# GATB/bcalm

Measured on AMD Instinct MI355X. Metric: distinct k-mers/s reads->unitigs k=31, higher is better.
Workload: dtype u64; 1 GPU; BASELINE config 3: synthetic 100000000 x 150 bp reads per GPU, k=31, abundance-min 2, 1% substitutions, 30x coverage; multi_gpu=single GPU, minimizer_size=16, log2_partitions=22

## Files before the change

bcalm_amd/csrc/host_glue.h:

```cpp
#pragma once

namespace {

template <int W>
int glue_join_impl(cdbg_ctx* c, bool sharded) {
    if (c->stage < 2) return fail(CDBG_E_STATE, "cdbg_glue before cdbg_compact");
    hipStream_t s = c->stream;
    const uint64_t NP = c->n_pieces;
    if (2 * NP >= 0x7FFFFFF0ULL) return fail(CDBG_E_INTERNAL, "too many pieces for 31-bit end ids (%llu)", (unsigned long long)NP);
    const uint32_t NS = (uint32_t)(2 * NP);
    Timer t; CK(t.start(s));
    CK(c->link.alloc(NS, false));
    HIPCK(hipMemsetAsync(c->link.p, 0xFF, (size_t)std::max<uint32_t>(NS, 1) * sizeof(uint32_t), s));
    HIPCK(hipMemsetAsync(c->dstats.p, 0, 32 * sizeof(uint64_t), s));
    HIPCK(hipMemsetAsync(c->derr.p, 0, 4 * sizeof(uint32_t), s));
    const uint32_t world = sharded ? (uint32_t)c->prm.world_size : 1u;
    const uint64_t n_mine = c->n_glog / world + (world > 1 ? (c->n_glog >> 6) + 1024 : 0);
    bool bucketed = (c->knobs.get("CDBG_GLUE_TABLE") == nullptr || c->direct_join) && c->n_glog > 0;
    if (bucketed && c->direct_join) {
        const uint64_t JB = 1ull << c->join_log_jb;
        JoinBucketParams bp{ c->jfill.p, c->jrecs.p, (uint32_t)JB, c->link.p, c->dstats.p, nullptr, nullptr, 0, nullptr };
        CDBG_LAUNCH((k_join_bucket<W>), std::min<uint64_t>((JB + 3) / 4, 256 * 16), JB_THREADS, s, bp);
    } else if (bucketed) {
        int log_jb = 0; while (((uint64_t)(JB_CAP / 2) << log_jb) < n_mine && log_jb < 26) ++log_jb;
        const uint64_t JB = 1ull << log_jb;
        CK(c->jfill.alloc(JB, false)); CK(c->jrecs.alloc(JB * JB_CAP * (W + 1), false));
        HIPCK(hipMemsetAsync(c->jfill.p, 0, JB * sizeof(uint32_t), s));
        JoinScatterParams sp{ c->glog_keys.p, c->glog_tag.p, c->n_glog, log_jb, c->jfill.p, c->jrecs.p, c->derr.p,
                              world - 1, world > 1 ? (uint32_t)c->prm.rank : 0u };
        CDBG_LAUNCH((k_join_scatter<W>), std::min<uint64_t>((c->n_glog + GLUE_THREADS - 1) / GLUE_THREADS, 1u << 16), GLUE_THREADS, s, sp);
        JoinBucketParams bp{ c->jfill.p, c->jrecs.p, (uint32_t)JB, c->link.p, c->dstats.p, nullptr, nullptr, 0, nullptr };
        CDBG_LAUNCH((k_join_bucket<W>), std::min<uint64_t>((JB + 3) / 4, 256 * 16), JB_THREADS, s, bp);
        HIPCK(hipStreamSynchronize(s));
        uint32_t e = 0; CK(read_u32(c->derr.p, &e));
        if (e == 8) {
            bucketed = false;
            HIPCK(hipMemsetAsync(c->link.p, 0xFF, (size_t)std::max<uint32_t>(NS, 1) * sizeof(uint32_t), s));
            HIPCK(hipMemsetAsync(c->dstats.p, 0, 32 * sizeof(uint64_t), s));
            HIPCK(hipMemsetAsync(c->derr.p, 0, 4 * sizeof(uint32_t), s));
        }
    }
    if (!bucketed && c->n_glog) {
        CK(glue_table_slots(n_mine + n_mine / 4 + 1024, &c->glue_cap));
        CK(c->glue_keys.alloc((uint64_t)c->glue_cap * W, false));
        CK(c->glue_a.alloc(c->glue_cap, false)); CK(c->glue_b.alloc(c->glue_cap, false)); CK(c->glue_conf.alloc(c->glue_cap, false));
        HIPCK(hipMemsetAsync(c->glue_keys.p, 0xFF, (uint64_t)c->glue_cap * W * sizeof(uint64_t), s));
        HIPCK(hipMemsetAsync(c->glue_a.p, 0, (uint64_t)c->glue_cap * sizeof(uint32_t), s));
        HIPCK(hipMemsetAsync(c->glue_b.p, 0, (uint64_t)c->glue_cap * sizeof(uint32_t), s));
        HIPCK(hipMemsetAsync(c->glue_conf.p, 0, (uint64_t)c->glue_cap * sizeof(uint32_t), s));
        GlueBuildParams bp{ c->glog_keys.p, c->glog_tag.p, c->n_glog, c->glue_keys.p, c->glue_a.p, c->glue_b.p, c->glue_conf.p, c->glue_cap - 1,
                            world - 1, world > 1 ? (uint32_t)c->prm.rank : 0u };
        CDBG_LAUNCH((k_glue_build<W>), std::min<uint64_t>((c->n_glog + GLUE_THREADS - 1) / GLUE_THREADS, MAX_GRID), GLUE_THREADS, s, bp);
        GlueResolveParams gp{};
        gp.keys = c->glue_keys.p; gp.a = c->glue_a.p; gp.b = c->glue_b.p; gp.conf = c->glue_conf.p;
        gp.cap = c->glue_cap; gp.W = W; gp.link = c->link.p; gp.stats = c->dstats.p;
        CDBG_LAUNCH(k_glue_resolve, std::min<uint64_t>((c->glue_cap + GLUE_THREADS - 1) / GLUE_THREADS, GLUE_RESOLVE_GRID), GLUE_THREADS, s, gp);
    }
    float ms = 0; CK(t.stop(&ms));
    CK(check_device_error(c, "glue join"));
    uint64_t gs = 0; CK(read_u64(c->dstats.p, &gs));
    c->n_join_local = gs; c->st.ms_glue = ms; c->joined = true;
    return CDBG_OK;
}


int glue_walk(cdbg_ctx* c, bool* done) {
    hipStream_t s = c->stream;
    const uint64_t NP = c->n_pieces, NS = 2 * NP;
    *done = false;
    if (!NP) return CDBG_OK;
    const uint64_t ucap = std::max<uint64_t>(NP, 1);
    const uint64_t ocap = std::max<uint64_t>(c->n_piece_bases, 1);
    CK(c->unitig_off.alloc(ucap, false)); CK(c->unitig_len.alloc(ucap, false)); CK(c->unitig_kc.alloc(ucap, false));
    CK(c->unitig_bases.alloc(ocap + 64, false));
    if (c->prm.all_abundance_counts) CK(c->unitig_ab.alloc(ocap, false));
    CK(c->rank_flag.alloc(4, true));
    CK(c->walk_rec.alloc(NS, false)); CK(c->walk_heads.alloc(NS, false)); CK(c->walk_hlen.alloc(NS, false)); CK(c->walk_hoff.alloc(NS, false));
    HIPCK(hipMemsetAsync(c->cursors.p + 2, 0, 2 * sizeof(uint64_t), s));
    HIPCK(hipMemsetAsync(c->dstats.p, 0, 32 * sizeof(uint64_t), s));
    HIPCK(hipMemsetAsync(c->derr.p, 0, 4 * sizeof(uint32_t), s));
    HIPCK(hipMemsetAsync(c->rank_flag.p, 0, sizeof(uint32_t), s));
    uint32_t max_steps = 4096;
    if (const char* e = c->knobs.get("CDBG_WALK_MAX")) max_steps = (uint32_t)strtoul(e, nullptr, 10);
    uint64_t* const n_heads = c->dstats.p + 6;
    WalkInitParams ip{ (uint32_t)NP, c->piece_n.p, c->piece_kc.p, c->piece_boff.p, c->link.p, c->walk_rec.p, c->walk_heads.p, n_heads, c->dstats.p + 4 };
    CDBG_LAUNCH(k_walk_init, (NP + WALK_PIECES - 1) / WALK_PIECES, WALK_THREADS, s, ip);
    const uint64_t spans = (NS + WALK_SPAN - 1) / WALK_SPAN, wave_grid = (spans + WALK_THREADS / 64 - 1) / (WALK_THREADS / 64);
    WalkMeasureParams mp{ c->walk_rec.p, c->walk_heads.p, n_heads, c->walk_hlen.p, max_steps, c->rank_flag.p };
    CDBG_LAUNCH(k_walk_measure, wave_grid, WALK_THREADS, s, mp);
    WalkPlaceParams pp{ n_heads, c->walk_hlen.p, c->walk_hoff.p, c->k, c->cursors.p + 2, c->cursors.p + 3, ucap, ocap, c->derr.p,
                        c->unitig_off.p, c->unitig_len.p };
    CDBG_LAUNCH(k_walk_place, spans, WALK_THREADS, s, pp);
    WalkCopyParams wp{};
    wp.k = c->k; wp.rec = c->walk_rec.p; wp.piece_bases = c->piece_bases.p;
    wp.heads = c->walk_heads.p; wp.n_heads = n_heads; wp.hlen = c->walk_hlen.p; wp.hoff = c->walk_hoff.p;
    wp.unitig_len = c->unitig_len.p; wp.unitig_kc = c->unitig_kc.p; wp.out = c->unitig_bases.p; wp.visited = c->dstats.p + 5;
    wp.piece_ab = c->prm.all_abundance_counts ? c->piece_ab.p : nullptr; wp.unitig_ab = c->unitig_ab.p; wp.error = c->derr.p;
    if (c->k >= 9) CDBG_LAUNCH(k_walk_copy<true>, wave_grid, WALK_THREADS, s, wp);
    else CDBG_LAUNCH(k_walk_copy<false>, wave_grid, WALK_THREADS, s, wp);
    HIPCK(hipStreamSynchronize(s));
    uint64_t d[2]; CK(read_u64(c->dstats.p + 4, d, 2));
    uint32_t gave_up = 0; CK(read_u32(c->rank_flag.p, &gave_up));
    if (gave_up || d[1] != d[0]) { c->walk_off = true; return CDBG_OK; }
    *done = true;
    return CDBG_OK;
}

template <int W>
int glue_impl(cdbg_ctx* c) {
    if (c->stage < 2) return fail(CDBG_E_STATE, "cdbg_glue before cdbg_compact");
    if ((c->prm.world_size > 1 || c->force_multi) && c->have_tr && !c->xchg_done && !c->joined) {
        if (!c->prm.emit_replicated && c->knobs.get("CDBG_GLUE_REPLICATED") == nullptr) {
            const int rc = glue_sharded<W>(c);
            if (rc != DG_FALLBACK) return rc;
        }
        CK(glue_exchange(c));
    }
    if (!c->joined) CK(glue_join_impl<W>(c, false));
    hipStream_t s = c->stream;
    const uint64_t NP = c->n_pieces;
    const uint32_t NS = (uint32_t)(2 * NP);
    const float ms_join = c->st.ms_glue;
    HostMarks hm;
    Timer t; CK(t.start(s));
    bool walked = false;
    if (c->prm.world_size <= 1 && !c->force_multi && !c->xchg_done && !c->walk_off && c->knobs.get("CDBG_GLUE_RANK") == nullptr) CK(glue_walk(c, &walked));
    if (walked) {
        { uint64_t cur[2]; CK(read_u64(c->cursors.p + 2, cur, 2)); c->n_unitigs = cur[0]; c->unitig_total = cur[1]; }
        CK(pack_unitigs(c));
        float ms_fin = 0; CK(t.stop(&ms_fin));
        hm.mark("glue: walk + copy");
        c->st.ms_glue = ms_join + ms_fin;
        CK(check_device_error(c, "glue"));
        c->joined = false;
        c->st.n_glue_joined = c->n_join_local; c->st.n_unitigs = c->n_unitigs; c->st.unitig_bases = c->unitig_total; c->st.n_walked_unitigs = c->n_unitigs;
        c->st.ms_total += c->st.ms_glue;
        c->stage = 3;
        return CDBG_OK;
    }
    DBuf<uint32_t>& flag = c->rank_flag; DBuf<uint4>& st_a = c->rank_a; DBuf<uint4>& st_b = c->rank_b;
    CK(st_a.alloc(NS, false)); CK(st_b.alloc(NS, false));
    CK(flag.alloc(4, true));
    HIPCK(hipMemsetAsync(c->dstats.p, 0, 32 * sizeof(uint64_t), s));
    HIPCK(hipMemsetAsync(c->derr.p, 0, 4 * sizeof(uint32_t), s));
    uint32_t* const link_p = c->link.p;

    uint64_t n_cycles_cut = 0;
    const uint32_t gridS = (NS + GLUE_THREADS - 1) / GLUE_THREADS;
    RankParams rp{};
    uint4* fa_st = nullptr;
    const uint2* st8 = nullptr; uint4* hinfo = nullptr;
    bool ranked = false;
    if (NS) {
        int max_rounds8 = 2; while ((1ull << (max_rounds8 - 1)) < NS) ++max_rounds8;
        Rank8Params r8{ NS, link_p, c->piece_n.p, reinterpret_cast<uint2*>(st_b.p), flag.p };
        CDBG_LAUNCH(k_rank8_init, gridS, GLUE_THREADS, s, r8);
        for (int r = 0; r < max_rounds8 && !ranked; ++r) {
            HIPCK(hipMemsetAsync(flag.p, 0, sizeof(uint32_t), s));
            CDBG_LAUNCH(k_rank8_jump, gridS, GLUE_THREADS, s, r8);
            HIPCK(hipStreamSynchronize(s));
            uint32_t ch = 0; CK(read_u32(flag.p, &ch));
            if (!ch) ranked = true;
        }
        if (ranked) { st8 = r8.a; hinfo = st_a.p; }
    }
    if (NS && !ranked) {
        int max_rounds = 2; while ((1ull << (max_rounds - 1)) < NS) ++max_rounds;
        for (int pass = 0; pass < 2; ++pass) {
            rp.n_states = NS; rp.link = link_p; rp.piece_n = c->piece_n.p;
            rp.st_a = st_a.p; rp.st_b = st_b.p; rp.changed = flag.p;
            CDBG_LAUNCH(k_rank_init, gridS, GLUE_THREADS, s, rp);
            bool converged = false;
            for (int r = 0; r < max_rounds; ++r) {
                HIPCK(hipMemsetAsync(flag.p, 0, sizeof(uint32_t), s));
                CDBG_LAUNCH(k_rank_jump, gridS, GLUE_THREADS, s, rp);
                std::swap(rp.st_a, rp.st_b);
                HIPCK(hipStreamSynchronize(s));
                uint32_t ch = 0; CK(read_u32(flag.p, &ch));
                if (!ch) { converged = true; break; }
            }
            fa_st = rp.st_a;
            if (converged) break;
            if (pass == 1) return fail(CDBG_E_INTERNAL, "list ranking did not converge after cutting cycles");
            HIPCK(hipMemsetAsync(flag.p, 0, sizeof(uint32_t), s));
            CutParams cu{ NS, rp.st_a, link_p, flag.p };
            CDBG_LAUNCH(k_cut_cycles, gridS, GLUE_THREADS, s, cu);
            HIPCK(hipStreamSynchronize(s));
            uint32_t nc = 0; CK(read_u32(flag.p, &nc)); n_cycles_cut += nc;
        }
    }
    if (NS && !st8) {
        uint4* const other = (fa_st == st_a.p) ? st_b.p : st_a.p;
        RankNarrowParams np{ NS, fa_st, reinterpret_cast<uint2*>(other) };
        CDBG_LAUNCH(k_rank_narrow, gridS, GLUE_THREADS, s, np);
        st8 = reinterpret_cast<const uint2*>(other); hinfo = fa_st;
    }
    const uint64_t ucap = std::max<uint64_t>(NP, 1);
    const uint64_t ocap = std::max<uint64_t>(c->n_piece_bases, 1);
    CK(c->unitig_off.alloc(ucap, false)); CK(c->unitig_len.alloc(ucap, false)); CK(c->unitig_kc.alloc(ucap, false));
    CK(c->unitig_bases.alloc(ocap + 64, false));
    if (c->prm.all_abundance_counts) CK(c->unitig_ab.alloc(ocap, false));
    HIPCK(hipMemsetAsync(c->cursors.p + 2, 0, 2 * sizeof(uint64_t), s));
    if (NS) {
        HeadParams hp{};
        hp.n_states = NS; hp.k = c->k; hp.link = link_p; hp.st = st8; hp.hinfo = hinfo;
        hp.unitig_off = c->unitig_off.p; hp.unitig_len = c->unitig_len.p; hp.unitig_kc = c->unitig_kc.p;
        hp.unitig_cap = ucap; hp.out_cap = ocap; hp.n_unitigs = c->cursors.p + 2; hp.out_cursor = c->cursors.p + 3; hp.error = c->derr.p;
        hp.own_lo = 0; hp.own_hi = NS;
        if (c->prm.world_size > 1 && !c->prm.emit_replicated && c->xchg_done) { hp.own_lo = (uint32_t)(2 * c->piece_lo); hp.own_hi = (uint32_t)(2 * c->piece_hi); }
        CDBG_LAUNCH(k_unitig_heads, (NS + HEADS_PER_WG - 1) / HEADS_PER_WG, GLUE_THREADS, s, hp);
        EmitParams ep{};
        ep.n_pieces = (uint32_t)NP; ep.k = c->k; ep.st = st8; ep.hinfo = hp.hinfo;
        ep.piece_n = c->piece_n.p; ep.piece_kc = c->piece_kc.p; ep.piece_boff = c->piece_boff.p; ep.piece_bases = c->piece_bases.p;
        ep.unitig_kc = c->unitig_kc.p; ep.out = c->unitig_bases.p;
        ep.piece_ab = c->prm.all_abundance_counts ? c->piece_ab.p : nullptr; ep.unitig_ab = c->unitig_ab.p;
        CDBG_LAUNCH(k_emit, (uint32_t)((NP + GLUE_THREADS - 1) / GLUE_THREADS), GLUE_THREADS, s, ep);
    }
    { uint64_t cur[2]; CK(read_u64(c->cursors.p + 2, cur, 2)); c->n_unitigs = cur[0]; c->unitig_total = cur[1]; }
    CK(pack_unitigs(c));
    float ms_fin = 0; CK(t.stop(&ms_fin));
    hm.mark("glue: rank + heads + emit");
    c->st.ms_glue = ms_join + ms_fin;
    CK(check_device_error(c, "glue"));
    c->joined = false;
    c->st.n_glue_joined = c->n_join_local; c->st.n_unitigs = c->n_unitigs; c->st.unitig_bases = c->unitig_total; c->st.n_cycles += n_cycles_cut;
    c->st.ms_total += c->st.ms_glue;
    c->stage = 3;
    return CDBG_OK;
}

struct UnitigView { uint64_t U; const uint64_t* off; const uint32_t* len; const uint8_t* bases; uint64_t total_bases; };

template <int W>
int links_build(cdbg_ctx* c, const UnitigView& v, DBuf<uint64_t>& link_off, DBuf<uint32_t>& link_to, uint64_t& n_links) {
    hipStream_t s = c->stream;
    const uint64_t U = v.U, NE = 2 * U;
    if (pow2_at_least(4 * U + 64) > (1ull << 30)) return fail(CDBG_E_INTERNAL, "too many unitigs (%llu) for the 30-bit slots of the link table", (unsigned long long)U);
    const uint32_t cap = (uint32_t)pow2_at_least(4 * U + 64);
    DBuf<uint64_t> lk_keys; DBuf<uint32_t> lk_cnt, lk_ends, end_slot, deg;
    CK(lk_keys.alloc((uint64_t)cap * W, false)); CK(lk_cnt.alloc((uint64_t)cap * 2, true));
    CK(lk_ends.alloc((uint64_t)cap * 2 * LINK_PER_FLAG, false)); CK(end_slot.alloc(NE, false)); CK(deg.alloc(NE, false));
    HIPCK(hipMemsetAsync(lk_keys.p, 0xFF, (uint64_t)cap * W * sizeof(uint64_t), s));
    CK(link_off.alloc(NE + 1, true));
    LinkParams lp{};
    lp.n_unitigs = U; lp.k = c->k; lp.unitig_off = v.off; lp.unitig_len = v.len; lp.bases = v.bases;
    lp.lk_keys = lk_keys.p; lp.lk_cnt = lk_cnt.p; lp.lk_ends = lk_ends.p; lp.lk_mask = cap - 1;
    lp.end_slot = end_slot.p; lp.deg = deg.p;
    n_links = 0;
    if (NE) {
        const uint64_t grid = (NE + LINK_THREADS - 1) / LINK_THREADS;
        CDBG_LAUNCH((k_link_insert<W>), grid, LINK_THREADS, s, lp);
        CDBG_LAUNCH(k_link_count, grid, LINK_THREADS, s, lp);
        const uint64_t nb = (NE + EXSCAN_BLOCK - 1) / EXSCAN_BLOCK;
        CK(c->exscan_tmp.alloc(nb + 1, false));
        const uint32_t* degp = deg.p;
        uint64_t* const loff = link_off.p;
        CDBG_LAUNCH(k_exscan_sums, nb, EXSCAN_THREADS, s, degp, c->exscan_tmp.p, NE);
        CDBG_LAUNCH(k_exscan_top, 1, EXSCAN_THREADS, s, c->exscan_tmp.p, nb, loff + NE);
        CDBG_LAUNCH(k_exscan_apply, nb, EXSCAN_THREADS, s, degp, (const uint64_t*)c->exscan_tmp.p, loff, NE);
        CK(read_u64(loff + NE, &n_links));
        CK(link_to.alloc(n_links, false));
        lp.link_off = link_off.p; lp.link_to = link_to.p;
        CDBG_LAUNCH(k_link_fill, grid, LINK_THREADS, s, lp);
        HIPCK(hipStreamSynchronize(s));
    }
    return CDBG_OK;
}
UnitigView resident_unitigs(cdbg_ctx* c) { return UnitigView{ c->n_unitigs, c->unitig_off.p, c->unitig_len.p, c->unitig_bases.p, c->unitig_total }; }
inline bool holds_a_share(const cdbg_ctx* c) { return (c->prm.world_size > 1 || c->force_multi) && !c->prm.emit_replicated; }

template <int W>
int links_build_sharded(cdbg_ctx* c) {
    hipStream_t s = c->stream;
    const int world = c->prm.world_size, me = c->prm.rank;
    if (!c->have_tr) return fail(CDBG_E_STATE, "cdbg_link on a sharded unitig set needs the transport");
    const uint64_t U = c->n_unitigs, NE = 2 * U;
    std::vector<uint64_t> all(world); const uint64_t mine = U;
    if (c->tr.all_gather_u64(c->tr.user, &mine, all.data(), 1) != 0) return fail(CDBG_E_INTERNAL, "transport all_gather_u64 failed");
    uint64_t tot = 0, base = 0; for (int r = 0; r < world; ++r) { if (r == me) base = tot; tot += all[r]; }
    c->unitig_id_base = base; c->unitig_id_total = tot;
    const uint64_t NA = 2 * tot;
    int rc = CDBG_OK;
    DBuf<uint64_t> lk_keys, end_keys, all_keys; DBuf<uint32_t> lk_cnt, lk_ends, end_slot, deg, end_meta, all_meta;
    uint32_t cap = 0;
    auto local = [&]() -> int {
        if (NA >= (1ull << 31) || pow2_at_least(2 * NA + 64) > (1ull << 30)) return fail(CDBG_E_INTERNAL, "too many unitigs (%llu) for the 30-bit slots of the link table", (unsigned long long)tot);
        cap = (uint32_t)pow2_at_least(2 * NA + 64);
        CK(end_keys.alloc(NE * W + 1, false)); CK(end_meta.alloc(NE + 1, false)); CK(all_keys.alloc(NA * W + 1, false)); CK(all_meta.alloc(NA + 1, false));
        CK(lk_keys.alloc((uint64_t)cap * W, false)); CK(lk_cnt.alloc((uint64_t)cap * 2, true));
        CK(lk_ends.alloc((uint64_t)cap * 2 * LINK_PER_FLAG, false)); CK(end_slot.alloc(NA + 1, false)); CK(deg.alloc(NE + 1, false));
        HIPCK(hipMemsetAsync(lk_keys.p, 0xFF, (uint64_t)cap * W * sizeof(uint64_t), s));
        CK(c->link_off.alloc(NE + 1, true));
        return CDBG_OK;
    };
    rc = local();
    CK(agree(c, rc, "links: buffers"));
    LinkParams lp{};
    lp.n_unitigs = U; lp.k = c->k; lp.unitig_off = c->unitig_off.p; lp.unitig_len = c->unitig_len.p; lp.bases = c->unitig_bases.p;
    lp.lk_keys = lk_keys.p; lp.lk_cnt = lk_cnt.p; lp.lk_ends = lk_ends.p; lp.lk_mask = cap - 1;
    lp.end_slot = end_slot.p; lp.deg = deg.p; lp.end_keys = end_keys.p; lp.end_meta = end_meta.p;
    lp.all_keys = all_keys.p; lp.all_meta = all_meta.p; lp.n_all_ends = NA; lp.e0 = 2 * base;
    const uint64_t grid = (NE + LINK_THREADS - 1) / LINK_THREADS;
    if (NE) CDBG_LAUNCH((k_link_describe<W>), grid, LINK_THREADS, s, lp);
    std::vector<uint64_t> roff(world), rcnt(world);
    { uint64_t o = 0; for (int r = 0; r < world; ++r) { roff[r] = o * 2 * W * 8; rcnt[r] = all[r] * 2 * W * 8; o += all[r]; } }
    if (!c->tr_ordered) HIPCK(hipStreamSynchronize(s));
    if (c->tr.all_gather_v(c->tr.user, end_keys.p, NE * W * 8, all_keys.p, roff.data(), rcnt.data()) != 0) return fail(CDBG_E_INTERNAL, "transport all_gather_v failed");
    { uint64_t o = 0; for (int r = 0; r < world; ++r) { roff[r] = o * 2 * 4; rcnt[r] = all[r] * 2 * 4; o += all[r]; if (r != me) c->comm_bytes += (NE + 2 * all[r]) * (uint64_t)(W * 8 + 4); } }
    if (c->tr.all_gather_v(c->tr.user, end_meta.p, NE * 4, all_meta.p, roff.data(), rcnt.data()) != 0) return fail(CDBG_E_INTERNAL, "transport all_gather_v failed");
    c->n_links = 0;
    auto join = [&]() -> int {
        if (NA) CDBG_LAUNCH((k_link_insert_described<W>), (NA + LINK_THREADS - 1) / LINK_THREADS, LINK_THREADS, s, lp);
        if (NE) {
            CDBG_LAUNCH(k_link_count, grid, LINK_THREADS, s, lp);
            const uint64_t nb = (NE + EXSCAN_BLOCK - 1) / EXSCAN_BLOCK;
            CK(c->exscan_tmp.alloc(nb + 1, false));
            const uint32_t* degp = deg.p; uint64_t* const loff = c->link_off.p;
            CDBG_LAUNCH(k_exscan_sums, nb, EXSCAN_THREADS, s, degp, c->exscan_tmp.p, NE);
            CDBG_LAUNCH(k_exscan_top, 1, EXSCAN_THREADS, s, c->exscan_tmp.p, nb, loff + NE);
            CDBG_LAUNCH(k_exscan_apply, nb, EXSCAN_THREADS, s, degp, (const uint64_t*)c->exscan_tmp.p, loff, NE);
            CK(read_u64(loff + NE, &c->n_links));
            CK(c->link_to.alloc(c->n_links, false));
            lp.link_off = c->link_off.p; lp.link_to = c->link_to.p;
            CDBG_LAUNCH(k_link_fill, grid, LINK_THREADS, s, lp);
        }
        HIPCK(hipStreamSynchronize(s));
        return CDBG_OK;
    };
    rc = join();
    CK(agree(c, rc, "links: join"));
    return CDBG_OK;
}

template <int W>
int link_impl(cdbg_ctx* c) {
    if (c->stage < 3) return fail(CDBG_E_STATE, "cdbg_link before cdbg_glue");
    if (holds_a_share(c)) CK(links_build_sharded<W>(c));
    else { CK(links_build<W>(c, resident_unitigs(c), c->link_off, c->link_to, c->n_links)); c->unitig_id_base = 0; c->unitig_id_total = c->n_unitigs; }
    c->linked = true;
    return CDBG_OK;
}

template <int W>
int verify_view(cdbg_ctx* c, const UnitigView& v, const uint64_t* link_off, const uint32_t* link_to, bool with_links, uint64_t* out) {
    hipStream_t s = c->stream;
    DBuf<uint64_t> d; CK(d.alloc(8, true));
    VerifyParams vp{ v.U, c->k, v.off, v.len, v.bases,
                     c->seg_off.p, c->seg_n.p, c->solid_keys.p, c->solid_cnt.p, c->n_local_parts, link_off, link_to, d.p };
    if (v.U) CDBG_LAUNCH((k_verify_unitig_kmers<W>), std::min<uint64_t>((v.U + 255) / 256, 1u << 16), 256, s, vp);
    CDBG_LAUNCH((k_verify_solid<W>), std::min<uint64_t>((c->n_local_parts + 255) / 256, 1u << 16), 256, s, vp);
    if (with_links && v.U) CDBG_LAUNCH(k_verify_maximal, (2 * v.U + 255) / 256, 256, s, vp);
    HIPCK(hipStreamSynchronize(s));
    CK(read_u64(d.p, out, 8));
    if (!with_links) out[6] = out[7] = ~0ull;
    return CDBG_OK;
}
template <int W>
int verify_edges_view(cdbg_ctx* c, const UnitigView& v, uint64_t n_links, uint64_t* out) {
    hipStream_t s = c->stream;
    const uint64_t n_home = c->st.n_solid;
    const uint64_t cap = pow2_at_least(3 * n_home + 1024);
    if (cap > (1ull << 32)) return fail(CDBG_E_NOMEM, "too many solid k-mers (%llu) for the 32-bit slots of the junction table", (unsigned long long)n_home);
    DBuf<uint64_t> jt_keys, d; DBuf<uint32_t> jt_cnt;
    CK(jt_keys.alloc(cap * W, false)); CK(jt_cnt.alloc(cap, false)); CK(d.alloc(4, true));
    HIPCK(hipMemsetAsync(jt_keys.p, 0xFF, cap * W * sizeof(uint64_t), s));
    HIPCK(hipMemsetAsync(jt_cnt.p, 0, cap * sizeof(uint32_t), s));
    VerifyEdgeParams ep{ c->k, c->seg_off.p, c->seg_n.p, c->solid_keys.p, c->solid_cnt.p, c->n_local_parts, jt_keys.p, jt_cnt.p, (uint32_t)(cap - 1), d.p };
    CDBG_LAUNCH((k_verify_edge_insert<W>), std::min<uint64_t>((c->n_local_parts + 255) / 256, 1u << 16), 256, s, ep);
    CDBG_LAUNCH(k_verify_edge_sum, std::min<uint64_t>((cap + 255) / 256, 1u << 16), 256, s, ep);
    HIPCK(hipStreamSynchronize(s));
    uint64_t r[4]; CK(read_u64(d.p, r, 4));
    if (r[2]) return fail(CDBG_E_INTERNAL, "junction table overflow in cdbg_verify_edges (%llu ends lost)", (unsigned long long)r[2]);
    out[0] = r[0]; out[1] = n_links; out[2] = 2 * (v.total_bases - v.U * (uint64_t)c->k); out[3] = r[1];
    return CDBG_OK;
}

template <int W>
int verify_impl(cdbg_ctx* c, uint64_t* out) {
    if (c->stage < 3) return fail(CDBG_E_STATE, "cdbg_verify before cdbg_glue");
    const bool sharded_set = holds_a_share(c);
    if (!sharded_set && !c->linked) CK(link_impl<W>(c));
    return verify_view<W>(c, resident_unitigs(c), c->link_off.p, c->link_to.p, !sharded_set, out);
}
template <int W>
int verify_edges_impl(cdbg_ctx* c, uint64_t* out) {
    if (c->stage < 3) return fail(CDBG_E_STATE, "cdbg_verify_edges before cdbg_glue");
    if (c->prm.world_size > 1 || c->force_multi) { out[0] = out[1] = out[2] = out[3] = ~0ull; return CDBG_OK; }
    if (!c->linked) CK(link_impl<W>(c));
    return verify_edges_view<W>(c, resident_unitigs(c), c->n_links, out);
}
template <int W>
int verify_unitigs_impl(cdbg_ctx* c, const char* bases, const uint64_t* off, uint64_t n, uint64_t* out) {
    if (c->stage < 1) return fail(CDBG_E_STATE, "cdbg_verify_unitigs before cdbg_count");
    if (c->prm.world_size > 1 || c->force_multi) return fail(CDBG_E_STATE, "cdbg_verify_unitigs needs the whole solid set on this rank");
    const uint64_t total = n ? off[n] : 0;
    std::vector<uint32_t> len(std::max<uint64_t>(n, 1));
    for (uint64_t i = 0; i < n; ++i) {
        if (off[i + 1] < off[i] || off[i + 1] - off[i] < (uint64_t)c->k || off[i + 1] - off[i] > 0xFFFFFFFFull) return fail(CDBG_E_PARAM, "unitig %llu: bad length", (unsigned long long)i);
        len[i] = (uint32_t)(off[i + 1] - off[i]);
    }
    for (uint64_t i = 0; i < total; ++i) if (!base_valid((uint8_t)bases[i])) return fail(CDBG_E_PARAM, "unitig base %llu is not one of ACGT", (unsigned long long)i);
    DBuf<uint64_t> d_off, l_off; DBuf<uint32_t> d_len, l_to; DBuf<uint8_t> d_bases;
    CK(d_off.alloc(n + 1, false)); CK(d_len.alloc(n, false)); CK(d_bases.alloc(total + 64, false));
    HIPCK(hipMemcpy(d_off.p, off, (n + 1) * sizeof(uint64_t), hipMemcpyHostToDevice));
    HIPCK(hipMemcpy(d_len.p, len.data(), std::max<uint64_t>(n, 1) * sizeof(uint32_t), hipMemcpyHostToDevice));
    if (total) HIPCK(hipMemcpy(d_bases.p, bases, total, hipMemcpyHostToDevice));
    const UnitigView v{ n, d_off.p, d_len.p, d_bases.p, total };
    uint64_t nl = 0;
    CK(links_build<W>(c, v, l_off, l_to, nl));
    CK(verify_view<W>(c, v, l_off.p, l_to.p, true, out));
    return verify_edges_view<W>(c, v, nl, out + 8);
}

}
```

bcalm_amd/csrc/k_walk.h:

```cpp
#pragma once
#include "k_glue.h"

namespace cdbg {

constexpr int WALK_THREADS = 256;
constexpr int WALK_PPT = 8;
constexpr int WALK_PIECES = WALK_THREADS * WALK_PPT;
constexpr int WALK_SPAN = 1024;
constexpr int WALK_SPT = WALK_SPAN / WALK_THREADS;

struct WalkInitParams { uint32_t n_pieces; const uint32_t* piece_n; const uint64_t* piece_kc; const uint64_t* piece_boff; const uint32_t* link;
                        uint4* rec; uint32_t* heads; uint64_t* n_heads; uint64_t* n_live; };
__global__ void __launch_bounds__(WALK_THREADS) k_walk_init(WalkInitParams P) {
    CDBG_SHARED uint32_t s_wn[WALK_THREADS / 64], s_wl[WALK_THREADS / 64]; CDBG_SHARED uint64_t s_base;
    const int tid = threadIdx.x, lane = tid & 63, wave = tid >> 6;
    const uint32_t p0 = blockIdx.x * (uint32_t)WALK_PIECES + (uint32_t)wave * (64u * WALK_PPT) + (uint32_t)lane;
    uint32_t hs[2 * WALK_PPT], at[WALK_PPT]; uint32_t run = 0, live = 0;
#pragma unroll
    for (int i = 0; i < WALK_PPT; ++i) {
        const uint32_t p = p0 + 64u * (uint32_t)i;
        hs[2 * i] = NONE32; hs[2 * i + 1] = NONE32;
        uint32_t cnt = 0;
        if (p < P.n_pieces) {
            const uint32_t n = P.piece_n[p];
            uint4 a, b; a.x = NONE32; a.y = NONE32; a.z = n; a.w = 0; b.x = 0; b.y = 0; b.z = 0; b.w = 0;
            if (n) {
                const uint64_t kc = P.piece_kc[p], bo = P.piece_boff[p];
                const uint2 l = reinterpret_cast<const uint2*>(P.link)[p];
                a.x = l.y; a.y = l.x;
                a.w = (uint32_t)kc; b.x = (uint32_t)(kc >> 32); b.y = (uint32_t)bo; b.z = (uint32_t)(bo >> 32);
                ++live;
                if (l.x == NONE32) { hs[2 * i] = 2 * p; ++cnt; }
                if (l.y == NONE32) { hs[2 * i + 1] = 2 * p + 1; ++cnt; }
            }
            P.rec[2 * (uint64_t)p] = a; P.rec[2 * (uint64_t)p + 1] = b;
        }
        const uint32_t incl = wave_incl_sum_u32(cnt);
        at[i] = run + incl - cnt;
        run += wave_readlane_u32(incl, 63);
    }
    const uint32_t lsum = wave_readlane_u32(wave_incl_sum_u32(live), 63);
    if (lane == 0) { s_wn[wave] = run; s_wl[wave] = lsum; }
    __syncthreads();
    uint32_t wbase = 0, tot = 0, ltot = 0;
    for (int w = 0; w < WALK_THREADS / 64; ++w) { if (w < wave) wbase += s_wn[w]; tot += s_wn[w]; ltot += s_wl[w]; }
    if (tid == 0) {
        s_base = tot ? atomic_add_u64(P.n_heads, (uint64_t)tot) : 0ull;
        if (ltot) atomic_add_u64(P.n_live, (uint64_t)ltot);
    }
    __syncthreads();
    uint32_t* const out = P.heads + s_base + wbase;
#pragma unroll
    for (int i = 0; i < WALK_PPT; ++i) {
        uint32_t j = at[i];
        if (hs[2 * i] != NONE32) out[j++] = hs[2 * i];
        if (hs[2 * i + 1] != NONE32) out[j] = hs[2 * i + 1];
    }
}

CDBG_DEV void walk_copy(const uint8_t* src, uint8_t* dst, uint32_t nb, uint32_t skip, bool fwd) {
    uint32_t i = skip;
    if (nb - skip >= 8u) {
        for (;;) {
            if (i + 8u > nb) { if (i == nb) break; i = nb - 8u; }
            const uint64_t w = fwd ? ld_unaligned_u64(src + i) : comp_ascii8_rev(ld_unaligned_u64(src + (nb - 8u - i)));
            st_unaligned_u64(dst + i, w);
            i += 8u;
        }
    } else {
        uint64_t w = 0; const uint32_t r = nb - skip;
        for (uint32_t j = 0; j < r; ++j) w |= (uint64_t)(fwd ? src[skip + j] : comp_ascii(src[nb - 1 - skip - j])) << (8 * j);
        if (r & 4u) { st_unaligned_u32(dst + i, (uint32_t)w); w >>= 32; i += 4u; }
        if (r & 2u) { st_unaligned_u16(dst + i, (uint16_t)w); w >>= 16; i += 2u; }
        if (r & 1u) dst[i] = (uint8_t)w;
    }
}

CDBG_DEV uint32_t walk_lane_rank(uint64_t mask, int lane) { return (uint32_t)__popcll(mask & ((1ULL << lane) - 1ULL)); }

struct WalkMeasureParams { const uint4* rec; const uint32_t* heads; const uint64_t* n_heads; uint32_t* hlen; uint32_t max_steps; uint32_t* giveup; };
__global__ void __launch_bounds__(WALK_THREADS) k_walk_measure(WalkMeasureParams P) {
    const int lane = threadIdx.x & 63;
    const uint64_t n_heads = *P.n_heads;
    const uint64_t wv = ((uint64_t)blockIdx.x * WALK_THREADS + threadIdx.x) >> 6;
    uint64_t next = wv * WALK_SPAN; const uint64_t end = next + WALK_SPAN < n_heads ? next + WALK_SPAN : n_heads;
    bool active = false; uint32_t e = 0, h = 0, len = 0, steps = 0; uint64_t idx = 0;
    for (;;) {
        const uint64_t need = __ballot(!active);
        if (next < end) {
            const uint64_t my = next + walk_lane_rank(need, lane);
            if (!active && my < end) { idx = my; h = P.heads[my]; e = h; len = 0; steps = 0; active = true; }
            next += (uint64_t)__popcll(need);
        }
        if (!__any(active)) break;
        if (active) {
            const uint4 a = P.rec[2 * (uint64_t)(e >> 1)];
            len += a.z;
            const uint32_t nx = (e & 1u) ? a.y : a.x;
            if (nx == NONE32) { P.hlen[idx] = e > (h ^ 1u) ? len : 0u; active = false; }
            else if (++steps > P.max_steps) { *P.giveup = 1u; P.hlen[idx] = 0u; active = false; }
            else e = nx;
        }
    }
}

struct WalkPlaceParams { const uint64_t* n_heads; uint32_t* hlen; uint64_t* hoff; int k; uint64_t* n_unitigs; uint64_t* out_cursor; uint64_t unitig_cap, out_cap; uint32_t* error;
                         uint64_t* unitig_off; uint32_t* unitig_len; };
__global__ void __launch_bounds__(WALK_THREADS) k_walk_place(WalkPlaceParams P) {
    CDBG_SHARED uint32_t s_wn[WALK_THREADS / 64]; CDBG_SHARED uint64_t s_wl[WALK_THREADS / 64];
    CDBG_SHARED uint64_t s_ubase, s_obase;
    const int tid = threadIdx.x, lane = tid & 63, wave = tid >> 6;
    const uint64_t n_heads = *P.n_heads;
    if ((uint64_t)blockIdx.x * WALK_SPAN >= n_heads) return;
    const uint64_t i0 = (uint64_t)blockIdx.x * WALK_SPAN + (uint64_t)tid * WALK_SPT;
    uint32_t kl[WALK_SPT]; uint32_t kn = 0; uint64_t ksum = 0;
#pragma unroll
    for (int i = 0; i < WALK_SPT; ++i) {
        kl[i] = i0 + i < n_heads ? P.hlen[i0 + i] : 0u;
        if (kl[i]) { ++kn; ksum += (uint64_t)kl[i] + (uint64_t)P.k - 1u; }
    }
    uint32_t icnt = kn; uint64_t isum = ksum;
#pragma unroll
    for (int d = 1; d < 64; d <<= 1) {
        const uint32_t c = __shfl_up(icnt, (unsigned)d); const uint64_t l = __shfl_up(isum, (unsigned)d);
        if (lane >= d) { icnt += c; isum += l; }
    }
    if (lane == 63) { s_wn[wave] = icnt; s_wl[wave] = isum; }
    __syncthreads();
    uint32_t my_i = icnt - kn, tot_n = 0; uint64_t my_o = isum - ksum, tot_l = 0;
    for (int w = 0; w < WALK_THREADS / 64; ++w) {
        if (w < wave) { my_i += s_wn[w]; my_o += s_wl[w]; }
        tot_n += s_wn[w]; tot_l += s_wl[w];
    }
    if (tid == 0 && tot_n) {
        s_ubase = atomic_add_u64(P.n_unitigs, (uint64_t)tot_n);
        s_obase = atomic_add_u64(P.out_cursor, tot_l);
        if (s_ubase + tot_n > P.unitig_cap || s_obase + tot_l > P.out_cap) *P.error = 4;
    }
    __syncthreads();
    if (!tot_n) return;
    const bool fits = s_ubase + tot_n <= P.unitig_cap && s_obase + tot_l <= P.out_cap;
    uint64_t uid = s_ubase + my_i, off = s_obase + my_o;
#pragma unroll
    for (int i = 0; i < WALK_SPT; ++i) {
        if (!kl[i]) continue;
        const uint32_t len = kl[i] + (uint32_t)P.k - 1u;
        P.hlen[i0 + i] = fits ? (uint32_t)uid + 1u : 0u; P.hoff[i0 + i] = off;
        if (fits) { P.unitig_off[uid] = off; P.unitig_len[uid] = len; }
        ++uid; off += (uint64_t)len;
    }
}

struct WalkCopyParams {
    int k; const uint4* rec; const uint8_t* piece_bases;
    const uint32_t* heads; const uint64_t* n_heads; const uint32_t* hlen; const uint64_t* hoff;
    const uint32_t* unitig_len; uint64_t* unitig_kc; uint8_t* out; uint64_t* visited;
    const uint32_t* piece_ab; uint32_t* unitig_ab;
    uint32_t* error;
};

struct WalkWin { uint64_t lo, hi, prev; uint32_t st; };
struct WalkDst { uint8_t* out; uint64_t u0; uint32_t ulen; uint32_t* error; uint32_t flushes; };

CDBG_DEV void wc_guard(WalkDst& D, uint64_t at, uint32_t bytes) {
#ifdef CDBG_HOSTSIM
    if (at < D.u0 || at + bytes > D.u0 + D.ulen) *D.error = 10;
#endif
}
CDBG_DEV void wc_st16(WalkDst& D, uint64_t at, uint64_t lo, uint64_t hi) {
    wc_guard(D, at, 16);
#ifdef CDBG_HOSTSIM
    if (at & 15u) *D.error = 10;
    __builtin_memcpy(D.out + at, &lo, 8); __builtin_memcpy(D.out + at + 8, &hi, 8);
#else
    uint4 v; v.x = (uint32_t)lo; v.y = (uint32_t)(lo >> 32); v.z = (uint32_t)hi; v.w = (uint32_t)(hi >> 32);
    *reinterpret_cast<uint4*>(D.out + at) = v;
#endif
}
CDBG_DEV void wc_st8(WalkDst& D, uint64_t at, uint64_t w) { wc_guard(D, at, 8); st_unaligned_u64(D.out + at, w); }
CDBG_DEV uint64_t wc_bytes8(uint64_t a, uint64_t b, uint32_t r) { return r == 0u ? a : r == 8u ? b : (a >> (8u * r)) | (b << (64u - 8u * r)); }
CDBG_DEV void wc_store_small(WalkDst& D, uint64_t at, uint64_t w0, uint64_t w1, uint64_t w2, uint32_t n) {
    wc_st8(D, at, w0);
    if (n >= 16u) { wc_st8(D, at + 8u, w1); if (n > 16u) wc_st8(D, at + n - 8u, wc_bytes8(w1, w2, n - 16u)); }
    else wc_st8(D, at + n - 8u, wc_bytes8(w0, w1, n - 8u));
}
CDBG_DEV void wc_flush(WalkWin& B, WalkDst& D, uint64_t cb) {
    ++D.flushes;
    if (cb >= D.u0) {
        wc_st16(D, cb, B.lo, B.hi);
        if (B.st == 1u) { const uint32_t h = 16u - ((uint32_t)D.u0 & 15u); wc_st8(D, D.u0, B.prev | (B.lo << (8u * h))); }
        B.prev = B.hi; B.st = 2u;
    } else {
        const uint32_t a = (uint32_t)(D.u0 - cb);
        if (a <= 8u) { wc_st8(D, D.u0, wc_bytes8(B.lo, B.hi, a)); if (a < 8u) wc_st8(D, cb + 8u, B.hi); B.prev = B.hi; B.st = 2u; }
        else { B.prev = B.hi >> (8u * (a - 8u)); B.st = 1u; }
    }
}
CDBG_DEV void wc_append(WalkWin& B, WalkDst& D, uint64_t pos, uint64_t w, uint32_t c) {
    const uint32_t s = (uint32_t)pos & 15u;
    if (s < 8u) { B.lo |= w << (8u * s); if (s) B.hi |= w >> (64u - 8u * s); }
    else {
        const uint32_t s8 = s - 8u;
        B.hi |= w << (8u * s8);
        if (s + c >= 16u) { wc_flush(B, D, pos - s); B.lo = s8 ? w >> (64u - 8u * s8) : 0ull; B.hi = 0; }
    }
}
CDBG_DEV void wc_finish(WalkWin& B, WalkDst& D, uint64_t end) {
    const uint32_t t = (uint32_t)end & 15u;
    if (B.st == 2u) {
        if (t >= 8u) { wc_st8(D, end - t, B.lo); if (t > 8u) wc_st8(D, end - 8u, wc_bytes8(B.lo, B.hi, t - 8u)); }
        else if (t) wc_st8(D, end - 8u, wc_bytes8(B.prev, B.lo, t));
    } else if (B.st == 1u) {
        const uint32_t h = 16u - ((uint32_t)D.u0 & 15u);
        wc_store_small(D, D.u0, B.prev | (B.lo << (8u * h)), (B.lo >> (64u - 8u * h)) | (B.hi << (8u * h)), B.hi >> (64u - 8u * h), h + t);
    } else {
        const uint32_t a = (uint32_t)D.u0 & 15u;
        wc_store_small(D, D.u0, wc_bytes8(B.lo, B.hi, a), B.hi >> (8u * a), 0, (uint32_t)(end - D.u0));
    }
}

template <bool CHUNKED>
__global__ void __launch_bounds__(WALK_THREADS) k_walk_copy(WalkCopyParams P) {
    const int lane = threadIdx.x & 63;
    const uint64_t n_heads = *P.n_heads;
    const uint64_t wv = ((uint64_t)blockIdx.x * WALK_THREADS + threadIdx.x) >> 6;
    uint64_t next = wv * WALK_SPAN; const uint64_t end = next + WALK_SPAN < n_heads ? next + WALK_SPAN : n_heads;
    bool active = false; uint32_t e = 0, koff = 0, uid = 0, seen = 0; uint64_t kc = 0, uoff = 0;
    WalkWin B{ 0, 0, 0, 0 }; WalkDst D{ P.out, 0, 0, P.error, 0 };
    for (;;) {
        const uint64_t need = __ballot(!active);
        if (next < end) {
            const uint64_t my = next + walk_lane_rank(need, lane);
            if (!active && my < end) {
                const uint32_t u1 = P.hlen[my];
                if (u1) {
                    uid = u1 - 1u; uoff = P.hoff[my]; e = P.heads[my]; koff = 0; kc = 0; active = true;
                    B.lo = 0; B.hi = 0; B.st = 0; D.u0 = uoff;
#ifdef CDBG_HOSTSIM
                    D.ulen = P.unitig_len[uid];
#endif
                }
            }
            next += (uint64_t)__popcll(need);
        }
        if (!__any(active)) { if (next < end) continue; break; }
        if (active) {
            const uint32_t p = e >> 1;
            const uint4 a = P.rec[2 * (uint64_t)p], b = P.rec[2 * (uint64_t)p + 1];
            const uint32_t n = a.z, nb = n + (uint32_t)P.k - 1u;
            const uint64_t boff = (uint64_t)b.y | ((uint64_t)b.z << 32);
            kc += (uint64_t)a.w | ((uint64_t)b.x << 32);
            const bool fwd = (e & 1u) == END_LEFT;
            const uint32_t skip = koff ? (uint32_t)P.k - 1u : 0u;
            if constexpr (CHUNKED) {
                const uint8_t* const src = P.piece_bases + boff;
                uint64_t pos = uoff + koff + skip;
                D.flushes = 0;
                for (uint32_t i = skip; i < nb;) {
                    const uint32_t c = nb - i < 8u ? nb - i : 8u, j = i + c - 8u;
                    const uint64_t w = fwd ? ld_unaligned_u64(src + j) : comp_ascii8_rev(ld_unaligned_u64(src + (nb - 8u - j)));
                    wc_append(B, D, pos, w >> (8u * (8u - c)), c);
                    pos += c; i += c;
                }
#ifdef CDBG_HOSTSIM
                if (const char* tf = getenv("CDBG_SIM_WALK_TRACE")) if (FILE* fp = fopen(tf, "a")) {
                    fprintf(fp, "%u %llu %u %u %d %u %d\n", uid, (unsigned long long)uoff, koff + skip, nb - skip, fwd ? 1 : 0, D.flushes,
                            ((e & 1u) ? a.y : a.x) == NONE32 ? 1 : 0);
                    fclose(fp);
                }
#endif
            } else {
#ifdef CDBG_HOSTSIM
                wc_guard(D, uoff + koff + skip, nb - skip);
#endif
                walk_copy(P.piece_bases + boff, P.out + uoff + koff, nb, skip, fwd);
            }
            if (P.piece_ab) {
                const uint32_t* sa = P.piece_ab + boff + (P.k - 1);
                uint32_t* da = P.unitig_ab + uoff + koff + (P.k - 1);
                if (fwd) { for (uint32_t t = 0; t < n; ++t) da[t] = sa[t]; }
                else { for (uint32_t t = 0; t < n; ++t) da[t] = sa[n - 1 - t]; }
            }
            koff += n; ++seen;
            const uint32_t nx = (e & 1u) ? a.y : a.x;
            if (nx == NONE32) {
                if constexpr (CHUNKED) wc_finish(B, D, uoff + koff + (uint32_t)P.k - 1u);
                P.unitig_kc[uid] = kc; active = false;
            }
            else e = nx;
        }
    }
    const uint64_t s64 = wave_sum_u64((uint64_t)seen);
    if (lane == 0 && s64) atomic_add_u64(P.visited, s64);
}

}
```

Baseline: 25.27 billion kmers/s.

## Inline short piece bases as 2-bit packed data in walk records

During walk init, pieces of up to 60 bases (k>=9, no abundance output) are packed into 2-bit form and stored in the 16-byte walk record, with a flag bit and 7 high k-count bits. The copy kernel then expands these inline bases, reverse-complementing in the 2-bit domain when needed, instead of doing scattered unaligned loads from piece_bases. The aim is to cut random global memory reads in the pointer-chasing walk, at the cost of extra bit-manipulation ALU work and more work in the init kernel.

New measurement: 25.46 billion kmers/s (median of 3 runs). About the same (+0.8%).

```diff
diff --git a/bcalm_amd/csrc/host_glue.h b/bcalm_amd/csrc/host_glue.h
--- a/bcalm_amd/csrc/host_glue.h
+++ b/bcalm_amd/csrc/host_glue.h
@@ -83,7 +83,9 @@
     uint32_t max_steps = 4096;
     if (const char* e = c->knobs.get("CDBG_WALK_MAX")) max_steps = (uint32_t)strtoul(e, nullptr, 10);
     uint64_t* const n_heads = c->dstats.p + 6;
-    WalkInitParams ip{ (uint32_t)NP, c->piece_n.p, c->piece_kc.p, c->piece_boff.p, c->link.p, c->walk_rec.p, c->walk_heads.p, n_heads, c->dstats.p + 4 };
+    const uint32_t inline_ok = c->k >= 9 && !c->prm.all_abundance_counts;
+    WalkInitParams ip{ (uint32_t)NP, c->piece_n.p, c->piece_kc.p, c->piece_boff.p, c->link.p, c->walk_rec.p, c->walk_heads.p, n_heads, c->dstats.p + 4,
+                       c->k, c->piece_bases.p, inline_ok };
     CDBG_LAUNCH(k_walk_init, (NP + WALK_PIECES - 1) / WALK_PIECES, WALK_THREADS, s, ip);
     const uint64_t spans = (NS + WALK_SPAN - 1) / WALK_SPAN, wave_grid = (spans + WALK_THREADS / 64 - 1) / (WALK_THREADS / 64);
     WalkMeasureParams mp{ c->walk_rec.p, c->walk_heads.p, n_heads, c->walk_hlen.p, max_steps, c->rank_flag.p };
diff --git a/bcalm_amd/csrc/k_walk.h b/bcalm_amd/csrc/k_walk.h
--- a/bcalm_amd/csrc/k_walk.h
+++ b/bcalm_amd/csrc/k_walk.h
@@ -9,8 +9,36 @@
 constexpr int WALK_SPAN = 1024;
 constexpr int WALK_SPT = WALK_SPAN / WALK_THREADS;
 
+constexpr uint32_t WALK_INLINE = 0x80000000u;
+constexpr uint32_t WALK_INLINE_NB = 60;
+constexpr int WALK_INLINE_KC_BITS = 39;
+CDBG_DEV uint64_t walk_pack8(uint64_t w) {
+    uint64_t x = (w >> 1) & 0x0303030303030303ull;
+    x = (x | (x >> 6)) & 0x000F000F000F000Full;
+    x = (x | (x >> 12)) & 0x000000FF000000FFull;
+    return (x | (x >> 24)) & 0xFFFFull;
+}
+CDBG_DEV uint64_t walk_expand8(uint32_t v) {
+    uint64_t x = v;
+    x = (x | (x << 24)) & 0x000000FF000000FFull;
+    x = (x | (x << 12)) & 0x000F000F000F000Full;
+    x = (x | (x << 6)) & 0x0303030303030303ull;
+    const uint64_t b0 = x & 0x0101010101010101ull, b1 = (x >> 1) & 0x0101010101010101ull, t = b1 & ~b0;
+    return 0x4040404040404040ull | (b0 << 1) | (b1 << 2) | (t << 4) | (t ^ 0x0101010101010101ull);
+}
+CDBG_DEV uint64_t walk_rev2(uint64_t x) {
+    x = ((x >> 2) & 0x3333333333333333ull) | ((x & 0x3333333333333333ull) << 2);
+    x = ((x >> 4) & 0x0F0F0F0F0F0F0F0Full) | ((x & 0x0F0F0F0F0F0F0F0Full) << 4);
+    return __builtin_bswap64(x);
+}
+CDBG_DEV void walk_shr128(uint64_t& lo, uint64_t& hi, uint32_t s) {
+    if (s >= 64u) { lo = hi >> (s - 64u); hi = 0; }
+    else if (s) { lo = (lo >> s) | (hi << (64u - s)); hi >>= s; }
+}
+
 struct WalkInitParams { uint32_t n_pieces; const uint32_t* piece_n; const uint64_t* piece_kc; const uint64_t* piece_boff; const uint32_t* link;
-                        uint4* rec; uint32_t* heads; uint64_t* n_heads; uint64_t* n_live; };
+                        uint4* rec; uint32_t* heads; uint64_t* n_heads; uint64_t* n_live;
+                        int k; const uint8_t* piece_bases; uint32_t inline_ok; };
 __global__ void __launch_bounds__(WALK_THREADS) k_walk_init(WalkInitParams P) {
     CDBG_SHARED uint32_t s_wn[WALK_THREADS / 64], s_wl[WALK_THREADS / 64]; CDBG_SHARED uint64_t s_base;
     const int tid = threadIdx.x, lane = tid & 63, wave = tid >> 6;
@@ -28,7 +56,24 @@
                 const uint64_t kc = P.piece_kc[p], bo = P.piece_boff[p];
                 const uint2 l = reinterpret_cast<const uint2*>(P.link)[p];
                 a.x = l.y; a.y = l.x;
-                a.w = (uint32_t)kc; b.x = (uint32_t)(kc >> 32); b.y = (uint32_t)bo; b.z = (uint32_t)(bo >> 32);
+                a.w = (uint32_t)kc;
+                const uint32_t nb = n + (uint32_t)P.k - 1u;
+                if (P.inline_ok && nb <= WALK_INLINE_NB && (kc >> WALK_INLINE_KC_BITS) == 0) {
+                    const uint8_t* const src = P.piece_bases + bo;
+                    uint64_t lo = 0, hi = 0;
+#pragma unroll
+                    for (uint32_t t = 0; t < (WALK_INLINE_NB - 1u) / 8u; ++t) {
+                        const bool whole = 8u * t + 8u <= nb;
+                        const uint64_t v = walk_pack8(ld_unaligned_u64(src + (whole ? 8u * t : nb - 8u)));
+                        if (whole) { if (t < 4u) lo |= v << (16u * t); else hi |= v << (16u * (t - 4u)); }
+                    }
+                    const uint64_t v = walk_pack8(ld_unaligned_u64(src + (nb - 8u)));
+                    const uint32_t s = 2u * (nb - 8u);
+                    if (s < 64u) { lo |= v << s; if (s > 48u) hi |= v >> (64u - s); }
+                    else hi |= v << (s - 64u);
+                    b.x = (uint32_t)lo; b.y = (uint32_t)(lo >> 32); b.z = (uint32_t)hi;
+                    b.w = (uint32_t)(hi >> 32) | ((uint32_t)(kc >> 32) << 24) | WALK_INLINE;
+                } else { b.x = (uint32_t)(kc >> 32); b.y = (uint32_t)bo; b.z = (uint32_t)(bo >> 32); }
                 ++live;
                 if (l.x == NONE32) { hs[2 * i] = 2 * p; ++cnt; }
                 if (l.y == NONE32) { hs[2 * i + 1] = 2 * p + 1; ++cnt; }
@@ -225,7 +270,7 @@
     const uint64_t n_heads = *P.n_heads;
     const uint64_t wv = ((uint64_t)blockIdx.x * WALK_THREADS + threadIdx.x) >> 6;
     uint64_t next = wv * WALK_SPAN; const uint64_t end = next + WALK_SPAN < n_heads ? next + WALK_SPAN : n_heads;
-    bool active = false; uint32_t e = 0, koff = 0, uid = 0, seen = 0; uint64_t kc = 0, uoff = 0;
+    bool active = false; uint32_t e = 0, koff = 0, uid = 0, seen = 0; uint64_t kc = 0;
     WalkWin B{ 0, 0, 0, 0 }; WalkDst D{ P.out, 0, 0, P.error, 0 };
     for (;;) {
         const uint64_t need = __ballot(!active);
@@ -234,8 +279,8 @@
             if (!active && my < end) {
                 const uint32_t u1 = P.hlen[my];
                 if (u1) {
-                    uid = u1 - 1u; uoff = P.hoff[my]; e = P.heads[my]; koff = 0; kc = 0; active = true;
-                    B.lo = 0; B.hi = 0; B.st = 0; D.u0 = uoff;
+                    uid = u1 - 1u; D.u0 = P.hoff[my]; e = P.heads[my]; koff = 0; kc = 0; active = true;
+                    B.lo = 0; B.hi = 0; B.st = 0;
 #ifdef CDBG_HOSTSIM
                     D.ulen = P.unitig_len[uid];
 #endif
@@ -248,43 +293,62 @@
             const uint32_t p = e >> 1;
             const uint4 a = P.rec[2 * (uint64_t)p], b = P.rec[2 * (uint64_t)p + 1];
             const uint32_t n = a.z, nb = n + (uint32_t)P.k - 1u;
+            const bool inl = CHUNKED && (b.w & WALK_INLINE);
             const uint64_t boff = (uint64_t)b.y | ((uint64_t)b.z << 32);
-            kc += (uint64_t)a.w | ((uint64_t)b.x << 32);
+            kc += (uint64_t)a.w | ((uint64_t)(inl ? (b.w >> 24) & 0x7Fu : b.x) << 32);
             const bool fwd = (e & 1u) == END_LEFT;
             const uint32_t skip = koff ? (uint32_t)P.k - 1u : 0u;
+            const uint32_t nx = (e & 1u) ? a.y : a.x;
+            if (P.piece_ab) {
+                const uint32_t* sa = P.piece_ab + boff + (P.k - 1);
+                uint32_t* da = P.unitig_ab + D.u0 + koff + (P.k - 1);
+                if (fwd) { for (uint32_t t = 0; t < n; ++t) da[t] = sa[t]; }
+                else { for (uint32_t t = 0; t < n; ++t) da[t] = sa[n - 1 - t]; }
+            }
             if constexpr (CHUNKED) {
                 const uint8_t* const src = P.piece_bases + boff;
-                uint64_t pos = uoff + koff + skip;
                 D.flushes = 0;
+                uint64_t lo = 0, hi = 0;
+                if (inl) {
+                    lo = (uint64_t)b.x | ((uint64_t)b.y << 32); hi = (uint64_t)b.z | ((uint64_t)(b.w & 0x00FFFFFFu) << 32);
+                    uint32_t sh = 2u * skip;
+                    if (!fwd) {
+                        const uint64_t r = walk_rev2(hi) ^ 0xAAAAAAAAAAAAAAAAull; hi = walk_rev2(lo) ^ 0xAAAAAAAAAAAAAAAAull; lo = r;
+                        sh += 2u * (64u - nb);
+                    }
+                    walk_shr128(lo, hi, sh);
+                }
                 for (uint32_t i = skip; i < nb;) {
-                    const uint32_t c = nb - i < 8u ? nb - i : 8u, j = i + c - 8u;
-                    const uint64_t w = fwd ? ld_unaligned_u64(src + j) : comp_ascii8_rev(ld_unaligned_u64(src + (nb - 8u - j)));
-                    wc_append(B, D, pos, w >> (8u * (8u - c)), c);
-                    pos += c; i += c;
+                    const uint32_t c = nb - i < 8u ? nb - i : 8u;
+                    uint64_t w;
+                    if (inl) {
+                        w = walk_expand8((uint32_t)lo & 0xFFFFu) & (~0ull >> (8u * (8u - c)));
+                        lo = (lo >> (2u * c)) | (hi << (64u - 2u * c)); hi >>= 2u * c;
+                    } else {
+                        const uint32_t j = i + c - 8u;
+                        w = (fwd ? ld_unaligned_u64(src + j) : comp_ascii8_rev(ld_unaligned_u64(src + (nb - 8u - j)))) >> (8u * (8u - c));
+                    }
+                    wc_append(B, D, D.u0 + koff + i, w, c);
+                    i += c;
                 }
 #ifdef CDBG_HOSTSIM
                 if (const char* tf = getenv("CDBG_SIM_WALK_TRACE")) if (FILE* fp = fopen(tf, "a")) {
-                    fprintf(fp, "%u %llu %u %u %d %u %d\n", uid, (unsigned long long)uoff, koff + skip, nb - skip, fwd ? 1 : 0, D.flushes,
-                            ((e & 1u) ? a.y : a.x) == NONE32 ? 1 : 0);
+                    fprintf(fp, "%u %llu %u %u %d %u %d", uid, (unsigned long long)D.u0, koff + skip, nb - skip, fwd ? 1 : 0, D.flushes,
+                            nx == NONE32 ? 1 : 0);
+                    if (getenv("CDBG_SIM_WALK_TRACE_INLINE")) fprintf(fp, " %d", inl ? 1 : 0);
+                    fprintf(fp, "\n");
                     fclose(fp);
                 }
 #endif
             } else {
 #ifdef CDBG_HOSTSIM
-                wc_guard(D, uoff + koff + skip, nb - skip);
-#endif
-                walk_copy(P.piece_bases + boff, P.out + uoff + koff, nb, skip, fwd);
-            }
-            if (P.piece_ab) {
-                const uint32_t* sa = P.piece_ab + boff + (P.k - 1);
-                uint32_t* da = P.unitig_ab + uoff + koff + (P.k - 1);
-                if (fwd) { for (uint32_t t = 0; t < n; ++t) da[t] = sa[t]; }
-                else { for (uint32_t t = 0; t < n; ++t) da[t] = sa[n - 1 - t]; }
+                wc_guard(D, D.u0 + koff + skip, nb - skip);
+#endif
+                walk_copy(P.piece_bases + boff, P.out + D.u0 + koff, nb, skip, fwd);
             }
             koff += n; ++seen;
-            const uint32_t nx = (e & 1u) ? a.y : a.x;
             if (nx == NONE32) {
-                if constexpr (CHUNKED) wc_finish(B, D, uoff + koff + (uint32_t)P.k - 1u);
+                if constexpr (CHUNKED) wc_finish(B, D, D.u0 + koff + (uint32_t)P.k - 1u);
                 P.unitig_kc[uid] = kc; active = false;
             }
             else e = nx;
```
